# FluxML/Flux3D.jl

Measured on AMD Instinct MI355X. Metric: chamfer_point_pairs_per_sec, higher is better.
Workload: dtype f32

## Files before the change

### flux3d.jl_amd/csrc/chamfer.hip

```cpp
#include <cmath>

#include "nn1_common.h"

using namespace fx3d;

#ifdef FX3D_PROBE
__device__ unsigned long long g_probe[4096 * 16];
#define FX3D_PROBE_MARK(k)                                                                   \
    do {                                                                                     \
        if (threadIdx.x == 0 && blockIdx.x < 4096) {                                         \
            g_probe[blockIdx.x * 16 + (k)] = __builtin_readcyclecounter();                   \
            if ((k) == 0) g_probe[blockIdx.x * 16 + 13] = wall_clock64();                    \
            if ((k) == 12) g_probe[blockIdx.x * 16 + 14] = wall_clock64();                   \
        }                                                                                    \
    } while (0)
__device__ unsigned long long g_probe2[256 * 16];
#define FX3D_PROBE_MARK2(k) do { if (threadIdx.x == 0 && blockIdx.x < 256) g_probe2[blockIdx.x * 16 + (k)] = __builtin_readcyclecounter(); } while (0)
__device__ unsigned long long g_probe3[16 * 16 * 8];
#define FX3D_PROBE_MARKW(k) do { if ((threadIdx.x & 63) == 0 && blockIdx.x < 16) g_probe3[(blockIdx.x * 16 + (threadIdx.x >> 6)) * 8 + (k)] = __builtin_readcyclecounter(); } while (0)
#else
#define FX3D_PROBE_MARK(k) do { } while (0)
#define FX3D_PROBE_MARK2(k) do { } while (0)
#define FX3D_PROBE_MARKW(k) do { } while (0)
#endif

namespace {

__device__ __forceinline__ void load4pts(const float *__restrict__ base, int p0, float (&px)[4],
                                         float (&py)[4], float (&pz)[4]) {
    const float4 *s4 = reinterpret_cast<const float4 *>(base + (size_t)p0 * 3);
    const float4 f0 = s4[0], f1 = s4[1], f2 = s4[2];
    px[0] = f0.x; py[0] = f0.y; pz[0] = f0.z;
    px[1] = f0.w; py[1] = f1.x; pz[1] = f1.y;
    px[2] = f1.z; py[2] = f1.w; pz[2] = f2.x;
    px[3] = f2.y; py[3] = f2.z; pz[3] = f2.w;
}

typedef _Float16 h8 __attribute__((ext_vector_type(8)));
typedef float f32x16 __attribute__((ext_vector_type(16)));
#ifndef FX3D_HFIFO
#define FX3D_HFIFO 5
#endif
constexpr int kHFifo = FX3D_HFIFO;
#ifndef FX3D_HRUNS_FROM
#define FX3D_HRUNS_FROM 16
#endif
constexpr int kHRunsFrom = FX3D_HRUNS_FROM;
constexpr int kScanU = 2;
#ifndef FX3D_HRUNCAP
#define FX3D_HRUNCAP 384
#endif
constexpr int kHRunCap = FX3D_HRUNCAP;
constexpr int kHItemCap = 64 * kHFifo > kHRunCap ? 64 * kHFifo : kHRunCap;
constexpr int kHFarCap = 64;
#ifndef FX3D_HBLKTRACK
#define FX3D_HBLKTRACK 1
#endif
constexpr bool kHBlkTrack = FX3D_HBLKTRACK != 0;
constexpr int kHIdBits = kHBlkTrack ? 7 : 6;
static_assert(kHChunkMax / (32 * kHLT) <= 64, "lane-tile ids live in the six (block ids: seven) low mantissa bits of the tracked keys");
constexpr float kKeyUp = kHBlkTrack ? 0x1.2p-16f : 0x1.2p-17f;
constexpr float kPadF16 = 65504.0f;
__device__ const unsigned short kHilbertCell[512] = {
    0, 1, 65, 64, 72, 73, 9, 8, 16, 24, 88, 80, 81, 89, 25, 17, 18, 26, 27, 19, 83, 91, 90, 82, 74, 10, 11, 75, 67, 3, 2, 66,
    130, 194, 195, 131, 139, 203, 202, 138, 146, 154, 155, 147, 211, 219, 218, 210, 209, 217, 153, 145, 144, 152, 216, 208, 200, 201, 137, 136, 128, 129, 193, 192,
    256, 257, 265, 264, 328, 329, 321, 320, 384, 448, 456, 392, 393, 457, 449, 385, 386, 450, 451, 387, 395, 459, 458, 394, 330, 322, 323, 331, 267, 259, 258, 266,
    274, 282, 283, 275, 339, 347, 346, 338, 402, 466, 467, 403, 411, 475, 474, 410, 409, 473, 465, 401, 400, 464, 472, 408, 344, 345, 337, 336, 272, 273, 281, 280,
    288, 296, 297, 289, 353, 361, 360, 352, 416, 480, 481, 417, 425, 489, 488, 424, 432, 496, 504, 440, 441, 505, 497, 433, 369, 368, 376, 377, 313, 312, 304, 305,
    306, 307, 315, 314, 378, 379, 371, 370, 434, 498, 506, 442, 443, 507, 499, 435, 427, 491, 490, 426, 418, 482, 483, 419, 355, 363, 362, 354, 290, 298, 299, 291,
    227, 235, 171, 163, 162, 170, 234, 226, 225, 224, 160, 161, 169, 168, 232, 233, 241, 240, 248, 249, 185, 184, 176, 177, 178, 242, 250, 186, 187, 251, 243, 179,
    115, 51, 59, 123, 122, 58, 50, 114, 113, 112, 120, 121, 57, 56, 48, 49, 41, 40, 104, 105, 97, 96, 32, 33, 34, 42, 106, 98, 99, 107, 43, 35,
    36, 44, 108, 100, 101, 109, 45, 37, 38, 39, 103, 102, 110, 111, 47, 46, 54, 55, 63, 62, 126, 127, 119, 118, 117, 53, 61, 125, 124, 60, 52, 116,
    180, 244, 252, 188, 189, 253, 245, 181, 182, 183, 191, 190, 254, 255, 247, 246, 238, 239, 175, 174, 166, 167, 231, 230, 229, 237, 173, 165, 164, 172, 236, 228,
    292, 300, 301, 293, 357, 365, 364, 356, 420, 484, 485, 421, 429, 493, 492, 428, 436, 500, 508, 444, 445, 509, 501, 437, 373, 372, 380, 381, 317, 316, 308, 309,
    310, 311, 319, 318, 382, 383, 375, 374, 438, 502, 510, 446, 447, 511, 503, 439, 431, 495, 494, 430, 422, 486, 487, 423, 359, 367, 366, 358, 294, 302, 303, 295,
    287, 286, 278, 279, 343, 342, 350, 351, 415, 479, 471, 407, 406, 470, 478, 414, 413, 477, 476, 412, 404, 468, 469, 405, 341, 349, 348, 340, 276, 284, 285, 277,
    269, 261, 260, 268, 332, 324, 325, 333, 397, 461, 460, 396, 388, 452, 453, 389, 390, 454, 462, 398, 399, 463, 455, 391, 327, 326, 334, 335, 271, 270, 262, 263,
    199, 198, 134, 135, 143, 142, 206, 207, 215, 223, 159, 151, 150, 158, 222, 214, 213, 221, 220, 212, 148, 156, 157, 149, 141, 205, 204, 140, 132, 196, 197, 133,
    69, 5, 4, 68, 76, 12, 13, 77, 85, 93, 92, 84, 20, 28, 29, 21, 22, 30, 94, 86, 87, 95, 31, 23, 15, 14, 78, 79, 71, 70, 6, 7,
};
constexpr size_t kHScratchBytes = (kHThreads / 64) * (32 * 8 + kHItemCap * 2 + 32 * 3 * 4) + 64 * 32;

__device__ __forceinline__ float vmin(float a, float b) {
    float r;
    asm("v_min_f32 %0, %1, %2" : "=v"(r) : "v"(a), "v"(b));
    return r;
}

__device__ __forceinline__ void split2h(float v, _Float16 &h, _Float16 &l) {
    h = (_Float16)v;
    l = (_Float16)(v - (float)h);
}

constexpr float kBetaC = 0x1.1p-18f;
constexpr float kBandB1 = 1.0f + 18.0f * kBetaC + 0x1p-20f;
constexpr float kBandA = 22.3f * kBetaC + 0x1p-19f;
__device__ __forceinline__ void make_pieces(float cx, float cy, float cz, h8 &p0, h8 &p1) {
    _Float16 hx, lx, hy, ly, hz, lz, n1, n2, n3;
    split2h(cx, hx, lx); split2h(cy, hy, ly); split2h(cz, hz, lz);
    const float n0 = ((cx * cx) + (cy * cy)) + (cz * cz);
    const float n = n0 + kBetaC * n0;
    n1 = (_Float16)n;
    const float r1 = n - (float)n1;
    n2 = (_Float16)r1;
    n3 = (_Float16)(r1 - (float)n2);
    const _Float16 z = (_Float16)0.0f;
    p0 = h8{hx, hx, lx, hy, hy, ly, hz, hz};
    p1 = h8{lz, n1, n2, n3, lx, ly, lz, z};
}

template <bool WANT_IDX, bool SPLITFUSE = false, bool PRUNE = false>
__global__ __launch_bounds__(kHThreads, 4) void nn1_f16_kernel(Nn1Params p) {
    extern __shared__ __attribute__((aligned(16))) float lds[];
    __shared__ __attribute__((aligned(16))) float red[4 * 4 * (kHThreads / 64) + 16];
    __shared__ int nfar[2];
    __shared__ unsigned short farlist[kHFarCap];
    constexpr int QB = (kHThreads / 64) * 32;

    const int L = blockIdx.x;
    const int per_cloud = p.tiles * p.nsplit;
    const bool by_xcd = 2 * p.B >= 8;
// ... 12 lines not shown
    const int NCm = NC - ctail;
    const float *__restrict__ qb = (dir ? p.y : p.x) + (size_t)b * NQ * 3;
    const float *__restrict__ cb = (dir ? p.x : p.y) + (size_t)b * NC * 3;
    int32_t *idx_out = dir ? p.idx_y : p.idx_x;
    float *dmin_out = dir ? p.dmin_y : p.dmin_x;

    const int tid = threadIdx.x, lane = tid & 63;
    const int wv = __builtin_amdgcn_readfirstlane(tid >> 6);
    const int jq = lane & 31, hh = lane >> 5;
    const int CH = p.chunk;
    const int tpb = dir ? p.tpb_y : p.tpb;
    h8 *imgp = reinterpret_cast<h8 *>(lds);
    float4 *imgf = reinterpret_cast<float4 *>(lds);
    unsigned long long *wres = reinterpret_cast<unsigned long long *>(lds + 8 * (CH + 64));
    unsigned short *witems = reinterpret_cast<unsigned short *>(wres + (kHThreads / 64) * 32);
    float *wq = reinterpret_cast<float *>(witems + (kHThreads / 64) * kHItemCap);
    unsigned long long *qres = wres + wv * 32;
    unsigned short *items = witems + wv * kHItemCap;
    float *qtab = wq + wv * 96;
    const bool vec = (reinterpret_cast<uintptr_t>(cb) & 15) == 0;
    const bool one_shot = NCm <= CH;
    if (tid == 0) { nfar[0] = 0; nfar[1] = 0; }
    float qpre[3];
    {
        const int q0i = (tile * tpb) * QB + wv * 32 + jq;
        const int qc0 = q0i < NQ ? q0i : NQ - 1;
#pragma unroll
        for (int d = 0; d < 3; ++d) qpre[d] = qb[(size_t)qc0 * 3 + d];
    }
    if constexpr (PRUNE) {
        unsigned int *zc = reinterpret_cast<unsigned int *>(wres);
        for (int i = tid; i < 1040 + 16 * 256; i += kHThreads) zc[i] = 0u;
        int *gb = reinterpret_cast<int *>(wq + (kHThreads / 64) * 96) + 64 * 8;
        for (int i = tid; i < kHGroupsMax * 8; i += kHThreads) gb[i] = (i & 4) ? (int)0x80000000 : 0x7fffffff;
    }
    FX3D_PROBE_MARK(0);

    const bool own_chunk_only = p.nsplit > 1 && (long long)split * CH + (long long)p.nsplit * CH >= NCm;
    const int s_lo = own_chunk_only ? split * CH : 0;
    const int SN = own_chunk_only ? (NCm - s_lo < CH ? NCm - s_lo : CH) : NC;
    const float *__restrict__ sb = cb + (size_t)s_lo * 3;
    const bool parked = one_shot || own_chunk_only;
    float mu[3], cinf = 0.0f, varmax = 0.0f;
    float bxlo[3] = {0.f, 0.f, 0.f}, bxhi[3] = {0.f, 0.f, 0.f};
    bool allfin = true;
    {
        float mn[3] = {INFINITY, INFINITY, INFINITY}, mx[3] = {-INFINITY, -INFINITY, -INFINITY}, sm3[3] = {0.f, 0.f, 0.f};
        float sqt = 0.0f;
        const float pil[3] = {sb[0], sb[1], sb[2]};
        const int nsweep = (SN + kHThreads - 1) / kHThreads;
        for (int i0 = 0; i0 < nsweep; i0 += 4) {
            P3 v[4];
#pragma unroll
            for (int e = 0; e < 4; ++e) {
                const int pt = (i0 + e) * kHThreads + tid;
                v[e] = *reinterpret_cast<const P3 *>(sb + (size_t)(pt < SN ? pt : SN - 1) * 3);
            }
#pragma unroll
            for (int e = 0; e < 4; ++e) {
                const int pt = (i0 + e) * kHThreads + tid;
                mn[0] = fminf(mn[0], v[e].x); mx[0] = fmaxf(mx[0], v[e].x);
                mn[1] = fminf(mn[1], v[e].y); mx[1] = fmaxf(mx[1], v[e].y);
                mn[2] = fminf(mn[2], v[e].z); mx[2] = fmaxf(mx[2], v[e].z);
                if (pt < SN) {
                    sm3[0] = sm3[0] + v[e].x; sm3[1] = sm3[1] + v[e].y; sm3[2] = sm3[2] + v[e].z;
                    if (parked) imgf[((pt >> 5) * 2) * 32 + (pt & 31)] = float4{v[e].x, v[e].y, v[e].z, 0.0f};
                }
// ... 32 lines not shown
#undef NN1_ROW_MAX
#undef NN1_ROW_SUM
            const float lo3[3] = {lo4.x, lo4.y, lo4.z}, hi3[3] = {hi4.x, hi4.y, hi4.z}, st3[3] = {st4.x, st4.y, st4.z};
            float m3[3], ci = 0.0f, vm = st4.w / fmaxf(0.25f * (float)SN, 1.0f);
            bool fin = true;
#pragma unroll
            for (int d = 0; d < 3; ++d) {
                const float lo = lo3[d], hi = hi3[d], st = st3[d];
                m3[d] = fminf(fmaxf(st / (float)SN, lo), hi);
                const float off = st / (float)SN - pil[d];
                vm = vm - off * off;
                ci = fmaxf(ci, fmaxf(hi - m3[d], m3[d] - lo));
                fin = fin && fabsf(st) < INFINITY;
            }
            if (lane == 0) {
                float4 *o4 = reinterpret_cast<float4 *>(red) + 4 * (kHThreads / 64);
                o4[0] = float4{m3[0], m3[1], m3[2], ci * 1.000001f};
                o4[1] = float4{vm, fin ? 1.0f : 0.0f, 0.0f, 0.0f};
                if (PRUNE) { o4[2] = float4{lo3[0], lo3[1], lo3[2], 0.0f}; o4[3] = float4{hi3[0], hi3[1], hi3[2], 0.0f}; }
            }
        }
        __syncthreads();
        {
            const float4 *o4 = reinterpret_cast<const float4 *>(red) + 4 * (kHThreads / 64);
            const float4 a = o4[0], b2 = o4[1];
            mu[0] = a.x; mu[1] = a.y; mu[2] = a.z; cinf = a.w;
            varmax = b2.x; allfin = b2.y != 0.0f;
            if (PRUNE) {
                const float4 l4 = o4[2], h4 = o4[3];
                bxlo[0] = l4.x; bxlo[1] = l4.y; bxlo[2] = l4.z; bxhi[0] = h4.x; bxhi[1] = h4.y; bxhi[2] = h4.z;
            }
        }
    }
    float rng = cinf;
    if (allfin && cinf < 1.0e16f && 3.0f * cinf * cinf > kRobustGate * varmax) {
        const float4 r = robust_range3<kHThreads, false>(sb, SN, parked, imgf, red, mu[0], mu[1], mu[2], cinf);
        mu[0] = r.x; mu[1] = r.y; mu[2] = r.z; rng = r.w;
    }
    const bool sane = allfin && cinf < 1.0e16f;
    float sc = 1.0f;
    if (sane && rng > 1.0e-30f) {
        int e;
        (void)frexpf(rng, &e);
        sc = ldexpf(1.0f, 7 - e);
    }
    auto uni = [](float v) { return __builtin_bit_cast(float, __builtin_amdgcn_readfirstlane(__builtin_bit_cast(int, v))); };
    mu[0] = uni(mu[0]); mu[1] = uni(mu[1]); mu[2] = uni(mu[2]); sc = uni(sc); rng = uni(rng); cinf = uni(cinf);
    const bool has_far = sane && rng < cinf;
    int fslot = 0;
    auto pieces = [&](float x, float y, float z, int pt, h8 &p0, h8 &p1) {
        const float sx = (x - mu[0]) * sc, sy = (y - mu[1]) * sc, sz = (z - mu[2]) * sc;
        if (!has_far) { make_pieces(sx, sy, sz, p0, p1); return; }
        const bool far = !(fmaxf(fmaxf(fabsf(sx), fabsf(sy)), fabsf(sz)) < 128.0f);
        make_pieces(far ? 0.f : sx, far ? 0.f : sy, far ? 0.f : sz, p0, p1);
        if (far) {
            p1[7] = (_Float16)kPadF16;
            const int f = atomicAdd(&nfar[fslot], 1);
            if (f < kHFarCap) farlist[f] = (unsigned short)pt;
        }
    };

    [[maybe_unused]] float4 *cs = nullptr, *qsw = nullptr;
    [[maybe_unused]] bool sorted_c = false;
    [[maybe_unused]] int qwlen = 0;
    [[maybe_unused]] float4 *boxes = nullptr;
    if constexpr (PRUNE) {
        cs = p.pscr + (size_t)blockIdx.x * p.pscr_stride;
        qsw = cs + kHChunkMax;
        boxes = reinterpret_cast<float4 *>(wq + (kHThreads / 64) * 96);
        unsigned int *ccnt = reinterpret_cast<unsigned int *>(wres);
        unsigned int *qtot = ccnt + 520;
        unsigned int *qwh = qtot + 520;
        const bool last_t = tile == (dir ? p.tiles_y : p.tiles_x) - 1;
        const int qw0 = tile * tpb * QB;
        const int qw1 = last_t || qw0 + tpb * QB > NQ ? NQ : qw0 + tpb * QB;
        qwlen = qw1 - qw0;
        const int cnt = NCm;
        const bool do_sort = sane && cnt >= 512;
        const bool sorted_q = do_sort && NQ <= 4 * kHThreads;
        P3 qv[4];
        if (sorted_q) {
#pragma unroll
            for (int e = 0; e < 4; ++e) {
                const int qp = 256 * wv + 64 * e + lane;
                qv[e] = *reinterpret_cast<const P3 *>(qb + (size_t)(qp < NQ ? qp : NQ - 1) * 3);
            }
        }
        FX3D_PROBE_MARK2(0);
        int *gbox = reinterpret_cast<int *>(boxes + 64 * 2);
        auto group_box = [&](int wrow, float x, float y, float z) {
            int *g = gbox + (wrow >> 5) * 8;
            atomicMin(g + 0, fkey((x - mu[0]) * sc)); atomicMin(g + 1, fkey((y - mu[1]) * sc)); atomicMin(g + 2, fkey((z - mu[2]) * sc));
            atomicMax(g + 4, fkey((x - mu[0]) * sc)); atomicMax(g + 5, fkey((y - mu[1]) * sc)); atomicMax(g + 6, fkey((z - mu[2]) * sc));
        };
        if (do_sort) {
            float4 cv[4];
#pragma unroll
            for (int e = 0; e < 4; ++e) {
                const int pt = e * kHThreads + tid;
                cv[e] = float4{0.f, 0.f, 0.f, 0.f};
                if (pt < cnt) cv[e] = imgf[((pt >> 5) * 2) * 32 + (pt & 31)];
            }
            FX3D_PROBE_MARK2(1);
            float inv[3], off[3], cfl[3], cfh[3];
#pragma unroll
            for (int d = 0; d < 3; ++d) {
                const float fr = has_far ? 0.125f * rng : 128.0f / sc;
                const float flo = fmaxf(bxlo[d], mu[d] - fr), fhi = fminf(bxhi[d], mu[d] + fr);
                inv[d] = fhi > flo ? 8.0f / (fhi - flo) : 0.0f;
                off[d] = -flo * inv[d];
                cfl[d] = flo; cfh[d] = fhi;
            }
            auto cell = [&](float x, float y, float z) -> unsigned int {
                const unsigned int ux = (unsigned int)(int)fminf(fmaxf(__builtin_fmaf(x, inv[0], off[0]), 0.0f), 7.0f);
                const unsigned int uy = (unsigned int)(int)fminf(fmaxf(__builtin_fmaf(y, inv[1], off[1]), 0.0f), 7.0f);
                const unsigned int uz = (unsigned int)(int)fminf(fmaxf(__builtin_fmaf(z, inv[2], off[2]), 0.0f), 7.0f);
                return ux | (uy << 3) | (uz << 6);
            };

            unsigned int ccr[4], qcr[4];
            auto count_cells = [&](bool valid, unsigned int t, auto &&add) -> unsigned int {
                unsigned int rank = 0u;
                bool mine = valid;
                const unsigned int tn = (unsigned int)__builtin_amdgcn_update_dpp((int)~t, (int)t, 0x111, 0xF, 0xF, false);
                if (__builtin_popcountll(__ballot(valid && t == tn)) >= 8) {
                    unsigned long long rem = __ballot(valid);
                    for (int it = 0; it < 12 && rem; ++it) {
                        const unsigned int t0 = (unsigned int)__builtin_amdgcn_readlane((int)t, __builtin_ctzll(rem));
                        const unsigned long long grp = __ballot(mine && t == t0);
                        rem &= ~grp;
                        if (__builtin_popcountll(grp) < 4) continue;
                        unsigned int base = 0u;
                        if ((int)lane == __builtin_ctzll(grp)) base = add(t0, (unsigned int)__builtin_popcountll(grp));
                        base = (unsigned int)__builtin_amdgcn_readlane((int)base, __builtin_ctzll(grp));
                        if (mine && t == t0) {
                            rank = base + __builtin_amdgcn_mbcnt_hi((unsigned int)(grp >> 32), __builtin_amdgcn_mbcnt_lo((unsigned int)grp, 0u));
                            mine = false;
                        }
                    }
                }
                if (mine) rank = add(t, 1u);
                return rank;
            };
#pragma unroll
            for (int e = 0; e < 4; ++e) {
                const int pt = e * kHThreads + tid;
                const unsigned int t = pt < cnt ? cell(cv[e].x, cv[e].y, cv[e].z) : 0u;
                ccr[e] = (t << 16) | count_cells(pt < cnt, t, [&](unsigned int c, unsigned int n) { return atomicAdd(&ccnt[c], n); });
            }
            int *qbb = reinterpret_cast<int *>(boxes + 64 * 2 + kHGroupsMax * 2 - 2);
            if (sorted_q) {
                int kl[3] = {0x7fffffff, 0x7fffffff, 0x7fffffff}, kh[3] = {(int)0x80000000, (int)0x80000000, (int)0x80000000};
#pragma unroll
                for (int e = 0; e < 4; ++e) {
                    const int qp = 256 * wv + 64 * e + lane;
                    if (qp < NQ) {
                        const int k3[3] = {fkey(qv[e].x), fkey(qv[e].y), fkey(qv[e].z)};
#pragma unroll
                        for (int d = 0; d < 3; ++d) { kl[d] = kl[d] < k3[d] ? kl[d] : k3[d]; kh[d] = kh[d] > k3[d] ? kh[d] : k3[d]; }
                    }
                }
#pragma unroll
                for (int d = 0; d < 3; ++d) {
                    int a = row_mm_key<false>(kl[d]), b2 = row_mm_key<true>(kh[d]);
                    a = imm<false>(a, dpp_keepi<0x142, 0xA>(a)); a = imm<false>(a, dpp_keepi<0x143, 0xC>(a));
                    b2 = imm<true>(b2, dpp_keepi<0x142, 0xA>(b2)); b2 = imm<true>(b2, dpp_keepi<0x143, 0xC>(b2));
                    if (lane == 63) { atomicMin(qbb + d, a); atomicMax(qbb + 4 + d, b2); }
                }
            }
            FX3D_PROBE_MARK2(2);
            __syncthreads();
            FX3D_PROBE_MARK2(3);
            float qinv[3] = {0.f, 0.f, 0.f}, qoff[3] = {0.f, 0.f, 0.f};
            if (sorted_q) {
                const float ext = fmaxf(fmaxf(cfh[0] - cfl[0], cfh[1] - cfl[1]), cfh[2] - cfl[2]);
#pragma unroll
                for (int d = 0; d < 3; ++d) {
                    const float ql = fkey_inv(qbb[d]), qh = fkey_inv(qbb[4 + d]);
                    const float grow = qh - ql > 4.0f * ext ? 0.25f * ext : ext;
                    const float lo = fmaxf(ql, cfl[d] - grow), hi = fminf(qh, cfh[d] + grow);
                    qinv[d] = hi > lo && hi - lo < INFINITY ? 8.0f / (hi - lo) : 0.0f;
                    qoff[d] = qinv[d] != 0.0f ? -lo * qinv[d] : 0.0f;
                }
            }
            auto qcell = [&](float x, float y, float z) -> unsigned int {
                const unsigned int ux = (unsigned int)(int)fminf(fmaxf(__builtin_fmaf(x, qinv[0], qoff[0]), 0.0f), 7.0f);
                const unsigned int uy = (unsigned int)(int)fminf(fmaxf(__builtin_fmaf(y, qinv[1], qoff[1]), 0.0f), 7.0f);
                const unsigned int uz = (unsigned int)(int)fminf(fmaxf(__builtin_fmaf(z, qinv[2], qoff[2]), 0.0f), 7.0f);
                return ux | (uy << 3) | (uz << 6);
            };
            auto curve_scan = [&](unsigned int *a) {
                unsigned int tc[8];
                {
                    const uint4 h = *reinterpret_cast<const uint4 *>(kHilbertCell + 8 * lane);
                    tc[0] = h.x & 0xffffu; tc[1] = h.x >> 16; tc[2] = h.y & 0xffffu; tc[3] = h.y >> 16;
                    tc[4] = h.z & 0xffffu; tc[5] = h.z >> 16; tc[6] = h.w & 0xffffu; tc[7] = h.w >> 16;
                }
                unsigned int c8[8], tot = 0u;
#pragma unroll
                for (int k = 0; k < 8; ++k) { c8[k] = a[tc[k]]; tot += c8[k]; }
                unsigned int inc = tot;
#pragma unroll
                for (int o = 1; o < 64; o <<= 1) {
                    const unsigned int v = __shfl_up(inc, o, 64);
                    if (lane >= o) inc += v;
                }
                unsigned int run = inc - tot;
#pragma unroll
                for (int k = 0; k < 8; ++k) { a[tc[k]] = run; run += c8[k]; }
            };
            if (wv == 0) curve_scan(ccnt);
            if (sorted_q) {
#pragma unroll
                for (int e = 0; e < 4; ++e) {
                    const int qp = 256 * wv + 64 * e + lane;
                    const unsigned int t = qp < NQ ? qcell(qv[e].x, qv[e].y, qv[e].z) : 0u;
                    qcr[e] = (t << 16) | count_cells(qp < NQ, t, [&](unsigned int c, unsigned int n) {
                                 const unsigned int sh = 16u * (c & 1u);
                                 const unsigned int old = atomicAdd(&qwh[wv * 256 + (c >> 1)], n << sh);
                                 atomicAdd(&qtot[c], n);
                                 return (old >> sh) & 0xffffu;
                             });
                }
            }
            FX3D_PROBE_MARK2(4);
            __syncthreads();
            FX3D_PROBE_MARK2(5);
#pragma unroll
            for (int e = 0; e < 4; ++e) {
                const int pt = e * kHThreads + tid;
                if (pt < cnt) {
                    const int pos = (int)(ccnt[ccr[e] >> 16] + (ccr[e] & 0xffffu));
                    imgf[((pos >> 5) * 2) * 32 + (pos & 31)] = float4{cv[e].x, cv[e].y, cv[e].z, __builtin_bit_cast(float, pt)};
                }
            }
            sorted_c = true;
            if (sorted_q) {
                if (wv == 1) {
                    curve_scan(qtot);
                } else if (wv >= 2 && wv < 6) {
                    const int w2 = tid - 128;
                    unsigned int run = 0u;
#pragma unroll
                    for (int w = 0; w < 16; ++w) {
                        const unsigned int v = qwh[w * 256 + w2];
                        qwh[w * 256 + w2] = run;
                        run += v;
                    }
                }
            }
            FX3D_PROBE_MARK2(6);
            __syncthreads();
            FX3D_PROBE_MARK2(7);
            if (sorted_q) {
#pragma unroll
                for (int e = 0; e < 4; ++e) {
                    const int qp = 256 * wv + 64 * e + lane;
                    if (qp < NQ) {
                        const unsigned int t = qcr[e] >> 16;
                        const int rank = (int)(qtot[t] + ((qwh[wv * 256 + (t >> 1)] >> (16u * (t & 1u))) & 0xffffu) + (qcr[e] & 0xffffu));
                        if (rank >= qw0 && rank < qw1) {
                            qsw[rank - qw0] = float4{qv[e].x, qv[e].y, qv[e].z, __builtin_bit_cast(float, qp)};
                            group_box(rank - qw0, qv[e].x, qv[e].y, qv[e].z);
                        }
                    }
                }
            }
        }
        if (!sorted_q) {
            for (int q0 = qw0 + wv * 64; q0 < qw1; q0 += kHThreads) {
                const int qp = q0 + lane;
                const P3 r = *reinterpret_cast<const P3 *>(qb + (size_t)(qp < qw1 ? qp : qw1 - 1) * 3);
                if (qp < qw1) qsw[qp - qw0] = float4{r.x, r.y, r.z, __builtin_bit_cast(float, qp)};
                const int kx = fkey((r.x - mu[0]) * sc), ky = fkey((r.y - mu[1]) * sc), kz = fkey((r.z - mu[2]) * sc);
                const int lx = row_mm_key<false>(kx), ly = row_mm_key<false>(ky), lz = row_mm_key<false>(kz);
                const int hx = row_mm_key<true>(kx), hy = row_mm_key<true>(ky), hz = row_mm_key<true>(kz);
                if ((lane & 15) == 0 && qp < qw1) {
                    int *g = gbox + ((qp - qw0) >> 5) * 8;
                    atomicMin(g + 0, lx); atomicMin(g + 1, ly); atomicMin(g + 2, lz);
                    atomicMax(g + 4, hx); atomicMax(g + 5, hy); atomicMax(g + 6, hz);
                }
            }
        }
        FX3D_PROBE_MARK2(8);
    }
    FX3D_PROBE_MARK(1);

    const float cm2 = 3.0f * (fminf(cinf * sc, 128.0f) * fminf(cinf * sc, 128.0f));
    float qr[3], da = 0.0f;
    float da_far = 0.0f;
    [[maybe_unused]] float dpr = INFINITY;
    bool qfin = true;
    int qi = 0;
    bool qok = true;
    h8 bq;
    double acc = 0.0;

    const int jfirst = split * CH, jstep = p.nsplit * CH;
    for (int j0 = jfirst; j0 < NCm; j0 += jstep) {
        const int cnt = (NCm - j0) < CH ? (NCm - j0) : CH;
        const int cnt_pad = (cnt + 32 * kHLT - 1) / (32 * kHLT) * (32 * kHLT);
        if (j0 > jfirst) __syncthreads();
        if constexpr (PRUNE) {
            for (int tl = tid >> 4; tl * 64 < cnt_pad + 64; tl += kHThreads / 16) {
                float4 r4[4];
#pragma unroll
                for (int k = 0; k < 4; ++k) {
                    const int pt = tl * 64 + k * 16 + (tid & 15);
                    r4[k] = float4{0.f, 0.f, 0.f, 0.f};
                    if (pt < cnt) r4[k] = imgf[((pt >> 5) * 2) * 32 + (pt & 31)];
                }
                float lo3[3] = {INFINITY, INFINITY, INFINITY}, hi3[3] = {-INFINITY, -INFINITY, -INFINITY};
#pragma unroll
                for (int k = 0; k < 4; ++k) {
                    const int pt = tl * 64 + k * 16 + (tid & 15), i0 = ((pt >> 5) * 2) * 32 + (pt & 31);
                    h8 p0, p1;
                    if (pt < cnt) {
                        pieces(r4[k].x, r4[k].y, r4[k].z, pt, p0, p1);
                        const int id = sorted_c ? __builtin_bit_cast(int, r4[k].w) : j0 + pt;
                        cs[pt] = float4{r4[k].x, r4[k].y, r4[k].z, __builtin_bit_cast(float, id)};
                        const float b3[3] = {(r4[k].x - mu[0]) * sc, (r4[k].y - mu[1]) * sc, (r4[k].z - mu[2]) * sc};
#pragma unroll
                        for (int d = 0; d < 3; ++d) { lo3[d] = vmin(lo3[d], b3[d]); hi3[d] = -vmin(-hi3[d], -b3[d]); }
                    } else {
                        make_pieces(0.f, 0.f, 0.f, p0, p1);
                        p1[7] = (_Float16)kPadF16;
                    }
                    imgp[i0] = p0;
                    imgp[i0 + 32] = p1;
                }
                float bl[3], bh[3];
#pragma unroll
                for (int d = 0; d < 3; ++d) { bl[d] = fkey_inv(row_mm_key<false>(fkey(lo3[d]))); bh[d] = fkey_inv(row_mm_key<true>(fkey(hi3[d]))); }
                if ((tid & 15) == 0 && tl < 64) {
                    boxes[tl * 2] = float4{bl[0], bl[1], bl[2], 0.0f};
                    boxes[tl * 2 + 1] = float4{bh[0], bh[1], bh[2], 0.0f};
                }
            }
        } else
        for (int pt = tid; pt < cnt_pad + 64; pt += kHThreads) {
            const int i0 = ((pt >> 5) * 2) * 32 + (pt & 31);
            h8 p0, p1;
            if (pt < cnt) {
                if (parked) {
                    const float4 r = imgf[i0];
                    pieces(r.x, r.y, r.z, pt, p0, p1);
                } else {
                    const P3 r = *reinterpret_cast<const P3 *>(cb + (size_t)(j0 + pt) * 3);
                    pieces(r.x, r.y, r.z, pt, p0, p1);
                }
            } else {
                make_pieces(0.f, 0.f, 0.f, p0, p1);
                p1[7] = (_Float16)kPadF16;
            }
            imgp[i0] = p0;
            imgp[i0 + 32] = p1;
        }
        __syncthreads();
        FX3D_PROBE_MARK(j0 == jfirst ? 2 : 6);
        FX3D_PROBE_MARKW(0);

        const int nf = nfar[fslot];
        if (tid == 0) nfar[fslot ^ 1] = 0;
        fslot ^= 1;
        const bool far_ok = nf <= kHFarCap;
        const bool last_tile = tile == (dir ? p.tiles_y : p.tiles_x) - 1;
        for (int tp = 0; tp < tpb || (last_tile && one_shot); ++tp) {
            if ((tile * tpb + tp) * QB >= NQ) break;
            if constexpr (PRUNE) {
                if (tp * QB + wv * 32 >= qwlen) continue;
            }
            if (j0 == jfirst) {
                qi = (tile * tpb + tp) * QB + wv * 32 + jq;
                if constexpr (PRUNE) {
                    const int wpos = tp * QB + wv * 32 + jq;
                    const float4 q4 = qsw[wpos < qwlen ? wpos : qwlen - 1];
                    qr[0] = q4.x; qr[1] = q4.y; qr[2] = q4.z;
                    qi = wpos < qwlen ? __builtin_bit_cast(int, q4.w) : NQ;
                } else if (tp == 0) {
#pragma unroll
                    for (int d = 0; d < 3; ++d) qr[d] = qpre[d];
                } else {
                    const int qc1 = qi < NQ ? qi : NQ - 1;
#pragma unroll
                    for (int d = 0; d < 3; ++d) qr[d] = qb[(size_t)qc1 * 3 + d];
                }
                float m0 = -2.0f * ((qr[0] - mu[0]) * sc), m1 = -2.0f * ((qr[1] - mu[1]) * sc), m2 = -2.0f * ((qr[2] - mu[2]) * sc);
                float S = (fabsf(m0) + fabsf(m1)) + fabsf(m2);
                float sq = 1.0f, fl_s = 0.0f;
                if (S >= 3.0e4f && S < 0x1p28f) {
                    int e;
                    (void)frexpf(S, &e);
                    sq = ldexpf(1.0f, 14 - e);
                    m0 *= sq; m1 *= sq; m2 *= sq; S *= sq;
                    fl_s = 0x1p-15f;
                }
                qok = S < 3.0e4f;
                qfin = fabsf(qr[0]) + fabsf(qr[1]) + fabsf(qr[2]) < INFINITY;
                const float qn = 0.25f * ((m0 * m0 + m1 * m1) + m2 * m2) / sq;
                da = kBandA * qn + 0x1p-24f * (S + 4.0f) + fl_s;
                {
                    const float c2 = sq * cm2;
                    da_far = 2.1f * kBetaC * c2 + 2.0f * kBetaC * sqrtf(qn * c2) + 0x1p-19f * qn + 0x1p-24f * (S + 4.0f) + fl_s;
                }
                if constexpr (PRUNE) {
                    dpr = qok && sq == 1.0f ? qn + 2.0f * kBetaC * (cm2 + qn) + 0x1p-23f * (S + 4.0f) : INFINITY;
                }
                _Float16 hx, lx, hy, ly, hz, lz;
                split2h(qok ? m0 : 0.f, hx, lx); split2h(qok ? m1 : 0.f, hy, ly); split2h(qok ? m2 : 0.f, hz, lz);
                const _Float16 one = (_Float16)sq, pad = (_Float16)kPadF16;
                bq = hh == 0 ? h8{hx, lx, hx, hy, ly, hy, hz, lz} : h8{hz, one, one, one, lx, ly, lz, pad};
                if (hh == 0) {
                    qres[jq] = ~0ull;
                    qtab[jq * 3 + 0] = qr[0]; qtab[jq * 3 + 1] = qr[1]; qtab[jq * 3 + 2] = qr[2];
                }
            }

            float tm = INFINITY, fk[kHFifo];
#pragma unroll
            for (int s = 0; s < kHFifo; ++s) fk[s] = INFINITY;
            const unsigned int keymask = ~((1u << kHIdBits) - 1u);

            static_assert(kHLT == 2, "the rotation below is written for lane tiles of two blocks");
            const int nblk = cnt_pad / 32;
            f32x16 zero;
#pragma unroll
            for (int r = 0; r < 16; ++r) zero[r] = 0.0f;
#define NN1_FOLD(ACC, FIRST)                                                                                         \
            {                                                                                                        \
                const float t0 = min3f(ACC[0], ACC[1], ACC[2]), t1 = min3f(ACC[3], ACC[4], ACC[5]);                  \
                const float t2 = min3f(ACC[6], ACC[7], ACC[8]), t3 = min3f(ACC[9], ACC[10], ACC[11]);                \
                const float t4 = min3f(ACC[12], ACC[13], ACC[14]);                                                   \
// ... 15 lines not shown
            __builtin_amdgcn_s_setprio(0);                                                                           \
            ISSUE = __builtin_amdgcn_mfma_f32_32x32x16_f16(an, bq, zero, 0, 0, 0);                                   \
            an = pa[(OFF) * 64];                                                                                     \
            __builtin_amdgcn_s_setprio(1);                                                                           \
            NN1_CLOSE(FOLD, ODD, lt)                                                                                 \
            if (ODD) ++lt;
            if constexpr (!PRUNE) {
            const h8 *pa = imgp + hh * 32 + jq;
            f32x16 acc0, acc1, acc2;
            h8 an = pa[0];
            acc0 = __builtin_amdgcn_mfma_f32_32x32x16_f16(an, bq, zero, 0, 0, 0); an = pa[1 * 64];
            acc1 = __builtin_amdgcn_mfma_f32_32x32x16_f16(an, bq, zero, 0, 0, 0); an = pa[2 * 64];
            pa += 3 * 64;
            int lt = 0;
            int nb = 2;
            for (; nb + 6 <= nblk; nb += 6) {
                NN1_STEP(acc2, acc0, 0, 0) NN1_STEP(acc0, acc1, 1, 1) NN1_STEP(acc1, acc2, 0, 2)
                NN1_STEP(acc2, acc0, 1, 3) NN1_STEP(acc0, acc1, 0, 4) NN1_STEP(acc1, acc2, 1, 5)
                pa += 6 * 64;
            }
            if (nblk - nb == 4) {
                NN1_STEP(acc2, acc0, 0, 0) NN1_STEP(acc0, acc1, 1, 1) NN1_STEP(acc1, acc2, 0, 2) NN1_STEP(acc2, acc0, 1, 3)
                NN1_CLOSE(acc1, 0, lt) NN1_CLOSE(acc2, 1, lt)
            } else if (nblk - nb == 2) {
                NN1_STEP(acc2, acc0, 0, 0) NN1_STEP(acc0, acc1, 1, 1)
                NN1_CLOSE(acc2, 0, lt) NN1_CLOSE(acc0, 1, lt)
            } else {
                NN1_CLOSE(acc0, 0, lt) NN1_CLOSE(acc1, 1, lt)
            }
            } else {
            const int nltp = nblk / kHLT;
            float bd = INFINITY;
            {
                const int4 *gq = reinterpret_cast<const int4 *>(boxes + 64 * 2) + (tp * (kHThreads / 64) + wv) * 2;
                const int4 gl = gq[0], gh = gq[1];
                const float qlx = fkey_inv(gl.x), qly = fkey_inv(gl.y), qlz = fkey_inv(gl.z);
                const float qhx = fkey_inv(gh.x), qhy = fkey_inv(gh.y), qhz = fkey_inv(gh.z);
                if (lane < nltp) {
                    const float4 lo = boxes[lane * 2], hi = boxes[lane * 2 + 1];
                    const float gx = fmaxf(fmaxf(lo.x - qhx, qlx - hi.x), 0.0f), gy = fmaxf(fmaxf(lo.y - qhy, qly - hi.y), 0.0f);
                    const float gz = fmaxf(fmaxf(lo.z - qhz, qlz - hi.z), 0.0f);
                    bd = (gx * gx + gy * gy) + gz * gz;
                }
            }
            const unsigned long long all_lt = nltp >= 64 ? ~0ull : (1ull << nltp) - 1ull;
            unsigned long long todo = all_lt, done = 0ull;
            if (sorted_c) {
                todo = __ballot(bd == 0.0f);
                if (!todo) {
                    const float bmin = wave_min_f(bd);
                    todo = bmin < INFINITY ? __ballot(bd == bmin) : all_lt;
                }
            }
            const h8 *pbase = imgp + hh * 32 + jq;
            for (int phase = 0; phase < 2; ++phase) {
                if (phase == 1) {
                    if (done == all_lt) break;
                    const float kb = fk[0];
                    const float bb = __builtin_fmaf(fabsf(kb), kKeyUp, kb);
                    const float dj = fminf(bb, __shfl_xor(bb, 32, 64)) + dpr;
                    const float ucut = wave_max_f(__builtin_fmaf(dj, 1.0f + 0x1p-9f, 0x1p-8f));
                    const bool keep = !(bd > ucut) || !(dj == dj);
                    todo = (__ballot(!(dj == dj)) ? all_lt : __ballot(keep)) & all_lt & ~done;
                    if (!todo) break;
                }
                done |= todo;
                unsigned long long mk = todo;
                int nrem = __builtin_popcountll(mk) - 1;
// ... 322 lines not shown
                        const float *src = cb + (size_t)jc * 3;
                        const float cc3[3] = {src[0], src[1], src[2]};
                        atomicMin(&qres[qs], ((unsigned long long)dist_key(sqd<3>(qq, cc3)) << 32) | (unsigned int)jc);
                    }
                }
            }
            FX3D_PROBE_MARK(tp == 0 ? 4 : 8);
            FX3D_PROBE_MARKW(tp == 0 ? 2 : 4);

            if (j0 + jstep >= NCm) {
                __builtin_amdgcn_s_waitcnt(0xc07f);
                __builtin_amdgcn_wave_barrier();
                if (hh == 0) {
                    const unsigned long long r = qres[jq];
                    const float dd = __builtin_bit_cast(float, (unsigned int)(r >> 32));
                    const int ii = (int)(unsigned int)r;
                    if (p.nsplit > 1) {
                        unsigned long long *gp = &p.gres[((size_t)split * 2 * p.B + c) * p.qstride + qi];
                        if (qi < NQ) {
                            if (SPLITFUSE) __hip_atomic_store(gp, r, __ATOMIC_RELAXED, __HIP_MEMORY_SCOPE_AGENT);
                            else *gp = r;
                        }
                    } else if (qi < NQ) {
                        if (WANT_IDX && idx_out) idx_out[(size_t)b * NQ + qi] = ii;
                        if (dmin_out) dmin_out[(size_t)b * NQ + qi] = dd;
                        acc += (double)dd;
                    }
                }
                __builtin_amdgcn_wave_barrier();
            }
        }
    }
    FX3D_PROBE_MARK(11);
    if (SPLITFUSE && p.nsplit > 1) {
        __shared__ int s_last;
        FX3D_PROBE_MARK2(10);
        asm volatile("s_waitcnt vmcnt(0)" ::: "memory");
        FX3D_PROBE_MARK2(11);
        __syncthreads();
        FX3D_PROBE_MARK2(12);
        const int ns = (NC + CH - 1) / CH < p.nsplit ? (NC + CH - 1) / CH : p.nsplit;
        if (tid == 0) {
            const unsigned int t = (unsigned int)c * (unsigned int)p.tiles + (unsigned int)tile;
            unsigned int *ctr = p.ticket + (t / 15u) * 16u + 1u + t % 15u;
            const unsigned int old = __hip_atomic_fetch_add(ctr, 1u, __ATOMIC_RELAXED, __HIP_MEMORY_SCOPE_AGENT);
            s_last = old == (unsigned int)ns - 1u;
            if (s_last) __hip_atomic_store(ctr, 0u, __ATOMIC_RELAXED, __HIP_MEMORY_SCOPE_AGENT);
            FX3D_PROBE_MARK2(13);
        }
        __syncthreads();
        if (!s_last) return;
        FX3D_PROBE_MARK(6);
        acc = 0.0;
        const int qend = (tile + 1) * tpb * QB < NQ ? (tile + 1) * tpb * QB : NQ;
        constexpr int kQ = 1, kS = 16;
        for (int q0 = tile * tpb * QB + tid; q0 < qend; q0 += kQ * kHThreads) {
          unsigned long long rr[kQ][kS];
#pragma unroll
          for (int u = 0; u < kQ; ++u)
#pragma unroll
            for (int sp = 0; sp < kS; ++sp) {
                const int q = q0 + u * kHThreads < qend ? q0 + u * kHThreads : q0;
                const int spc = sp < ns ? sp : ns - 1;
                rr[u][sp] = __hip_atomic_load(&p.gres[((size_t)spc * 2 * p.B + c) * p.qstride + q], __ATOMIC_RELAXED, __HIP_MEMORY_SCOPE_AGENT);
            }
#ifdef FX3D_PROBE
// ... 57 lines not shown
#pragma unroll
            for (int e = 0; e < 4; ++e) o[e] = p.gres[((size_t)(sp + e < ns ? sp + e : 0) * 2 * p.B + c) * p.qstride + qi];
#pragma unroll
            for (int e = 0; e < 4; ++e) r = o[e] < r ? o[e] : r;
        }
        const float dd = __builtin_bit_cast(float, (unsigned int)(r >> 32));
        int32_t *idx_out = dir ? p.idx_y : p.idx_x;
        float *dmin_out = dir ? p.dmin_y : p.dmin_x;
        if (idx_out) idx_out[(size_t)b * NQ + qi] = (int)(unsigned int)r;
        if (dmin_out) dmin_out[(size_t)b * NQ + qi] = dd;
        acc = (double)dd;
    }
    if (p.partials) {
        __shared__ double sm[kThreads / 64];
        const double tot = block_sum<kThreads>(acc, sm);
        if (!p.ticket) {
            if (threadIdx.x == 0) p.partials[(size_t)c * tiles_f + blockIdx.x] = tot;
            return;
        }
        if (threadIdx.x < 64) {
            const FinalizeArgs fa{reinterpret_cast<unsigned long long *>(p.partials), p.ticket, p.nvalid, p.B, tiles_f, p.tiles_x, p.tiles_y,
                                  p.sums_out, p.loss_out, p.N, p.M, p.Bg, p.w1, p.w2};
            (void)fused_finalize_wave0(fa, (size_t)c * tiles_f + blockIdx.x, tot, (int)threadIdx.x);
        }
    }
}

}

namespace fx3d {

size_t nn1_f16_lds_bytes(int chunk) { return (size_t)chunk * 8 * sizeof(float) + kHScratchBytes; }

constexpr size_t kHBoxBytes = 64 * 2 * sizeof(float4) + kHGroupsMax * 32;

template <bool WANT_IDX>
static fx3d_status launch_f16(const Nn1Params &p, int grid, size_t lds_bytes, hipStream_t st) {
    void (*const kfn)(Nn1Params) = p.pscr ? &nn1_f16_kernel<WANT_IDX, false, true>
                                   : p.fuse_split ? &nn1_f16_kernel<WANT_IDX, true> : &nn1_f16_kernel<WANT_IDX, false>;
    const size_t box = p.pscr ? kHBoxBytes : 0;
    const fx3d_status arc = ensure_dynamic_lds(reinterpret_cast<const void *>(kfn), (int)(nn1_f16_lds_bytes(kHChunkMax) + box), "nn1_f16_kernel");
    if (arc != FX3D_OK) return arc;
    hipLaunchKernelGGL(kfn, dim3(grid), dim3(kHThreads), lds_bytes + box, st, p);
    FX3D_LAUNCH_CHECK();
    return FX3D_OK;
}

fx3d_status nn1_f16_launch(const Nn1Params &p, int grid, size_t lds_bytes, hipStream_t st) {
    return p.idx_x || p.idx_y ? launch_f16<true>(p, grid, lds_bytes, st) : launch_f16<false>(p, grid, lds_bytes, st);
}

fx3d_status nn1_split_finalize_launch(const Nn1Params &p, int tiles_f, hipStream_t st) {
    hipLaunchKernelGGL(nn1_split_finalize_kernel, dim3(tiles_f, 2 * p.B), dim3(kThreads), 0, st, p, tiles_f);
    FX3D_LAUNCH_CHECK();
    return FX3D_OK;
}

}
```

### flux3d.jl_amd/csrc/chamfer_host.hip

```cpp
#include <cmath>
#include <cstdlib>

#include "nn1_common.h"

using namespace fx3d;

namespace {

struct FinalizeParams {
    const double *partials;
    int B, tiles, tiles_x, tiles_y;
    double *sums;
    float *loss;
    int N, M, D;
    long long Bg;
    float w1, w2;
};

__global__ __launch_bounds__(kThreads) void chamfer_finalize_partials_kernel(FinalizeParams f) {
    __shared__ double sm[kThreads / 64];
    double tot[2];
    for (int dir = 0; dir < 2; ++dir) {
        const int nt = dir ? f.tiles_y : f.tiles_x;
        const long long n = (long long)f.B * nt;
// ... 142 lines not shown
                t = t > thr ? t : thr;
                const long long tmax = tiles_a > tiles_b ? tiles_a : tiles_b;
                t += 1.0 * (double)((2ll * B * tmax + ncu - 1) / ncu - 1);
                if (t < bt - 1e-9) { bt = t; pl.tpb = ta; pl.tpb_y = tb; }
            }
    }
    const bool fold = b_split == 1 && maxc <= b_chunk;
    auto ntiles = [&](int nq, int tpb) {
        const int per = 512 * tpb;
        int t = ceil_div(nq, per);
        if (fold && t > 1 && nq - (t - 1) * per <= kHTail) --t;
        return t;
    };
    pl.tiles_x = ntiles(N, pl.tpb);
    pl.tiles_y = ntiles(M, pl.tpb_y);
    pl.tiles = pl.tiles_x > pl.tiles_y ? pl.tiles_x : pl.tiles_y;
    pl.grid = clouds8 * 8 * pl.tiles * pl.nsplit;
    if (2 * B < 8) pl.grid = 2 * B * pl.tiles * pl.nsplit;
    return pl;
}

Nn1Kernel plan_kernel(const Plan &pl, int D) {
    if (D != 2 && D != 3) return NN1_GENERIC;
    return pl.variant == 3 ? NN1_F16 : pl.variant == 4 ? NN1_TINY : NN1_SMALL_D;
}
const char *plan_kernel_name(const Plan &pl, int D) {
    static const char *const names[] = {"generic", "small_d", "tiny", "f16"};
    return names[plan_kernel(pl, D)];
}

int prune_rows_per_block(const Plan &pl, int N, int M, int D) {
    const int maxc = N > M ? N : M;
    if (plan_kernel(pl, D) != NN1_F16 || pl.nsplit != 1 || pl.tail != 0 || maxc > pl.chunk || maxc < 1024 || !opt(OPT_NN1_PRUNE)) return 0;
    if ((pl.tpb > pl.tpb_y ? pl.tpb : pl.tpb_y) * 16 + 2 > kHGroupsMax - 1) return 0;
    if ((pl.tpb < pl.tpb_y ? pl.tpb : pl.tpb_y) < 2) return 0;
    return kHChunkMax + (pl.tpb > pl.tpb_y ? pl.tpb : pl.tpb_y) * 512 + kHTail;
}

struct Workspace {
    int tiles;
    size_t sums, gres, need, pscr, total;
};
Workspace workspace_layout(const Plan &pl, int N, int M, int B, int D) {
    Workspace w{};
    const int maxq = N > M ? N : M;
    w.tiles = pl.nsplit > 1 ? ceil_div(maxq, kThreads) : pl.tiles;
    w.sums = (size_t)2 * B * w.tiles * sizeof(double);
    w.gres = w.sums + 2 * sizeof(double);
    w.need = w.gres + (pl.nsplit > 1 ? (size_t)pl.nsplit * 2 * B * maxq * sizeof(unsigned long long) : 0);
    w.pscr = (w.need + 255) & ~(size_t)255;
    const size_t ps = (size_t)prune_rows_per_block(pl, N, M, D) * pl.grid * sizeof(float4);
    w.total = ps ? w.pscr + ps : w.need;
    return w;
}

constexpr long long kSplitFuseMax = 255;

fx3d_status run_nn1(Nn1Params p, int D, const Plan &pl, hipStream_t st) {
    p.tiles = pl.tiles; p.tiles_x = pl.tiles_x; p.tiles_y = pl.tiles_y; p.chunk = pl.chunk;
    p.tpb = pl.tpb; p.tpb_y = pl.tpb_y;
    p.tail = pl.tail;
    p.nsplit = p.gres ? pl.nsplit : 1;
    p.fuse_split = p.gres && p.ticket ? 1 : 0;
    p.pscr_stride = p.pscr ? prune_rows_per_block(pl, p.N, p.M, D) : 0;
    if (!p.pscr_stride) p.pscr = nullptr;
    const Nn1Kernel k = plan_kernel(pl, D);
    ProfileScope prof("nn1", st);
// ... 144 lines not shown
```

### flux3d.jl_amd/csrc/nn1_common.h

```cpp
#pragma once
#include "fx3d_common.h"

namespace fx3d {

constexpr int kThreads = 256;
constexpr int kTile = 32;
constexpr int kChunkMax = 4096;

struct Nn1Params {
    const float *x;
    const float *y;
    int N, M, B;
    int32_t *idx_x, *idx_y;
    float *dmin_x, *dmin_y;
    double *partials;
    int tiles;
    int tiles_x, tiles_y;
    int chunk;
    int tpb;
    int tpb_y;
    unsigned int *ticket;
    unsigned int nvalid;
    double *sums_out;
    float *loss_out;
// ... 26 lines not shown
    for (int d = 1; d < DIM; ++d) {
        float t = q[d] - c[d];
        s = s + t * t;
    }
    return s;
}

__device__ __forceinline__ bool fless(float a, float b) { return (a < b) || (b != b && a == a); }
__device__ __forceinline__ unsigned int dist_key(float d) { return d != d ? 0x7fc00000u : __builtin_bit_cast(unsigned int, d); }

template <int DIM>
__device__ __forceinline__ void nn1_scan_isless(const float (&q)[DIM], const float *__restrict__ cb, int NC, float &best, int &bi) {
    float c0[DIM];
#pragma unroll
    for (int d = 0; d < DIM; ++d) c0[d] = cb[d];
    best = sqd<DIM>(q, c0);
    bi = 0;
    for (int j = 1; j < NC; ++j) {
        float cc[DIM];
#pragma unroll
        for (int d = 0; d < DIM; ++d) cc[d] = cb[(size_t)j * DIM + d];
        const float dd = sqd<DIM>(q, cc);
        if (fless(dd, best)) { best = dd; bi = j; }
    }
}

constexpr int kHThreads = 1024;
#ifndef FX3D_HLT
#define FX3D_HLT 2
#endif
constexpr int kHLT = FX3D_HLT;
constexpr int kHChunkMax = 4096;
constexpr int kHTail = 64;
constexpr int kHGroupsMax = 8 * 16 + 2 + 1;

constexpr int kTyThreads = 256;
constexpr int kTyQ = 16;
constexpr int kTySl = 16;
constexpr int kTyG = 16;

__device__ __forceinline__ float chamfer_loss_from_sums(double sa, double sb, int N, int M, int D,
                                                        long long Bg, float w1, float w2) {
    const float dA = (float)(sa / ((double)D * (double)N * (double)Bg)) * 3.0f;
    const float dB = (float)(sb / ((double)D * (double)M * (double)Bg)) * 3.0f;
    return (w1 * dA) + (w2 * dB);
}

#if defined(__HIP_DEVICE_COMPILE__) && !defined(__gfx950__)
#error "nn1_common.h: the relaxed-atomic + s_waitcnt hand-off between blocks is validated on gfx950 only (see the note above)"
#endif
struct FinalizeArgs {
    unsigned long long *pp;
    unsigned int *ticket;
    unsigned int nvalid;
    int B, stride, tiles_x, tiles_y;
    double *sums_out;
    float *loss_out;
    int N, M;
    long long Bg;
    float w1, w2;
};
__device__ __forceinline__ int fused_finalize_wave0(const FinalizeArgs &f, size_t slot, double tot, int lane) {
    int last = 0;
    if (lane == 0) {
        __hip_atomic_store(&f.pp[slot], __builtin_bit_cast(unsigned long long, tot), __ATOMIC_RELAXED, __HIP_MEMORY_SCOPE_AGENT);
        asm volatile("s_waitcnt vmcnt(0)" ::: "memory");
        const unsigned int old = __hip_atomic_fetch_add(f.ticket, 1u, __ATOMIC_RELAXED, __HIP_MEMORY_SCOPE_AGENT);
// ... 34 lines not shown
```

Measured before the change: 14580 billion.

## Compute per-half-wave query boxes with lane reductions instead of LDS atomics

```diff
diff --git a/flux3d.jl_amd/csrc/chamfer.hip b/flux3d.jl_amd/csrc/chamfer.hip
--- a/flux3d.jl_amd/csrc/chamfer.hip
+++ b/flux3d.jl_amd/csrc/chamfer.hip
@@ -22,6 +22,11 @@
 #define FX3D_PROBE_MARK(k) do { } while (0)
 #define FX3D_PROBE_MARK2(k) do { } while (0)
 #define FX3D_PROBE_MARKW(k) do { } while (0)
+#endif
+#ifdef FX3D_PROBE_STOP
+#define FX3D_PROBE_STOP_AT(k) do { if (FX3D_PROBE_STOP == (k)) return; } while (0)
+#else
+#define FX3D_PROBE_STOP_AT(k) do { } while (0)
 #endif
 
 namespace {
@@ -87,6 +92,18 @@
     return r;
 }
 
+template <bool MAX>
+__device__ __forceinline__ int half_mm_key(int k) {
+    k = row_mm_key<MAX>(k);
+    return imm<MAX>(__builtin_amdgcn_readlane(k, 0), __builtin_amdgcn_readlane(k, 16));
+}
+
+__device__ __forceinline__ float vmax(float a, float b) {
+    float r;
+    asm("v_max_f32 %0, %1, %2" : "=v"(r) : "v"(a), "v"(b));
+    return r;
+}
+
 __device__ __forceinline__ void split2h(float v, _Float16 &h, _Float16 &l) {
     h = (_Float16)v;
     l = (_Float16)(v - (float)h);
@@ -165,7 +182,7 @@
         unsigned int *zc = reinterpret_cast<unsigned int *>(wres);
         for (int i = tid; i < 1040 + 16 * 256; i += kHThreads) zc[i] = 0u;
         int *gb = reinterpret_cast<int *>(wq + (kHThreads / 64) * 96) + 64 * 8;
-        for (int i = tid; i < kHGroupsMax * 8; i += kHThreads) gb[i] = (i & 4) ? (int)0x80000000 : 0x7fffffff;
+        if (tid < 8) gb[tid] = (tid & 4) ? (int)0x80000000 : 0x7fffffff;
     }
     FX3D_PROBE_MARK(0);
 
@@ -264,6 +281,7 @@
             }
         }
     }
+    FX3D_PROBE_STOP_AT(1);
     float rng = cinf;
     if (allfin && cinf < 1.0e16f && 3.0f * cinf * cinf > kRobustGate * varmax) {
         const float4 r = robust_range3<kHThreads, false>(sb, SN, parked, imgf, red, mu[0], mu[1], mu[2], cinf);
@@ -319,12 +337,6 @@
             }
         }
         FX3D_PROBE_MARK2(0);
-        int *gbox = reinterpret_cast<int *>(boxes + 64 * 2);
-        auto group_box = [&](int wrow, float x, float y, float z) {
-            int *g = gbox + (wrow >> 5) * 8;
-            atomicMin(g + 0, fkey((x - mu[0]) * sc)); atomicMin(g + 1, fkey((y - mu[1]) * sc)); atomicMin(g + 2, fkey((z - mu[2]) * sc));
-            atomicMax(g + 4, fkey((x - mu[0]) * sc)); atomicMax(g + 5, fkey((y - mu[1]) * sc)); atomicMax(g + 6, fkey((z - mu[2]) * sc));
-        };
         if (do_sort) {
             float4 cv[4];
 #pragma unroll
@@ -380,7 +392,7 @@
                 const unsigned int t = pt < cnt ? cell(cv[e].x, cv[e].y, cv[e].z) : 0u;
                 ccr[e] = (t << 16) | count_cells(pt < cnt, t, [&](unsigned int c, unsigned int n) { return atomicAdd(&ccnt[c], n); });
             }
-            int *qbb = reinterpret_cast<int *>(boxes + 64 * 2 + kHGroupsMax * 2 - 2);
+            int *qbb = reinterpret_cast<int *>(boxes + 64 * 2);
             if (sorted_q) {
                 int kl[3] = {0x7fffffff, 0x7fffffff, 0x7fffffff}, kh[3] = {(int)0x80000000, (int)0x80000000, (int)0x80000000};
 #pragma unroll
@@ -403,6 +415,7 @@
             FX3D_PROBE_MARK2(2);
             __syncthreads();
             FX3D_PROBE_MARK2(3);
+            FX3D_PROBE_STOP_AT(2);
             float qinv[3] = {0.f, 0.f, 0.f}, qoff[3] = {0.f, 0.f, 0.f};
             if (sorted_q) {
                 const float ext = fmaxf(fmaxf(cfh[0] - cfl[0], cfh[1] - cfl[1]), cfh[2] - cfl[2]);
@@ -458,6 +471,7 @@
             FX3D_PROBE_MARK2(4);
             __syncthreads();
             FX3D_PROBE_MARK2(5);
+            FX3D_PROBE_STOP_AT(3);
 #pragma unroll
             for (int e = 0; e < 4; ++e) {
                 const int pt = e * kHThreads + tid;
@@ -484,6 +498,7 @@
             FX3D_PROBE_MARK2(6);
             __syncthreads();
             FX3D_PROBE_MARK2(7);
+            FX3D_PROBE_STOP_AT(4);
             if (sorted_q) {
 #pragma unroll
                 for (int e = 0; e < 4; ++e) {
@@ -491,10 +506,7 @@
                     if (qp < NQ) {
                         const unsigned int t = qcr[e] >> 16;
                         const int rank = (int)(qtot[t] + ((qwh[wv * 256 + (t >> 1)] >> (16u * (t & 1u))) & 0xffffu) + (qcr[e] & 0xffffu));
-                        if (rank >= qw0 && rank < qw1) {
-                            qsw[rank - qw0] = float4{qv[e].x, qv[e].y, qv[e].z, __builtin_bit_cast(float, qp)};
-                            group_box(rank - qw0, qv[e].x, qv[e].y, qv[e].z);
-                        }
+                        if (rank >= qw0 && rank < qw1) qsw[rank - qw0] = float4{qv[e].x, qv[e].y, qv[e].z, __builtin_bit_cast(float, qp)};
                     }
                 }
             }
@@ -504,19 +516,12 @@
                 const int qp = q0 + lane;
                 const P3 r = *reinterpret_cast<const P3 *>(qb + (size_t)(qp < qw1 ? qp : qw1 - 1) * 3);
                 if (qp < qw1) qsw[qp - qw0] = float4{r.x, r.y, r.z, __builtin_bit_cast(float, qp)};
-                const int kx = fkey((r.x - mu[0]) * sc), ky = fkey((r.y - mu[1]) * sc), kz = fkey((r.z - mu[2]) * sc);
-                const int lx = row_mm_key<false>(kx), ly = row_mm_key<false>(ky), lz = row_mm_key<false>(kz);
-                const int hx = row_mm_key<true>(kx), hy = row_mm_key<true>(ky), hz = row_mm_key<true>(kz);
-                if ((lane & 15) == 0 && qp < qw1) {
-                    int *g = gbox + ((qp - qw0) >> 5) * 8;
-                    atomicMin(g + 0, lx); atomicMin(g + 1, ly); atomicMin(g + 2, lz);
-                    atomicMax(g + 4, hx); atomicMax(g + 5, hy); atomicMax(g + 6, hz);
-                }
             }
         }
         FX3D_PROBE_MARK2(8);
     }
     FX3D_PROBE_MARK(1);
+    FX3D_PROBE_STOP_AT(5);
 
     const float cm2 = 3.0f * (fminf(cinf * sc, 128.0f) * fminf(cinf * sc, 128.0f));
     float qr[3], da = 0.0f;
@@ -534,7 +539,13 @@
         const int cnt_pad = (cnt + 32 * kHLT - 1) / (32 * kHLT) * (32 * kHLT);
         if (j0 > jfirst) __syncthreads();
         if constexpr (PRUNE) {
-            for (int tl = tid >> 4; tl * 64 < cnt_pad + 64; tl += kHThreads / 16) {
+            if (tid >= kHThreads - 64) {
+                const int pt = cnt_pad + lane, i0 = ((pt >> 5) * 2) * 32 + (pt & 31);
+                const _Float16 z = (_Float16)0.0f;
+                imgp[i0] = h8{z, z, z, z, z, z, z, z};
+                imgp[i0 + 32] = h8{z, z, z, z, z, z, z, (_Float16)kPadF16};
+            }
+            for (int tl = tid >> 4; tl * 64 < cnt_pad; tl += kHThreads / 16) {
                 float4 r4[4];
 #pragma unroll
                 for (int k = 0; k < 4; ++k) {
@@ -553,7 +564,7 @@
                         cs[pt] = float4{r4[k].x, r4[k].y, r4[k].z, __builtin_bit_cast(float, id)};
                         const float b3[3] = {(r4[k].x - mu[0]) * sc, (r4[k].y - mu[1]) * sc, (r4[k].z - mu[2]) * sc};
 #pragma unroll
-                        for (int d = 0; d < 3; ++d) { lo3[d] = vmin(lo3[d], b3[d]); hi3[d] = -vmin(-hi3[d], -b3[d]); }
+                        for (int d = 0; d < 3; ++d) { lo3[d] = vmin(lo3[d], b3[d]); hi3[d] = vmax(hi3[d], b3[d]); }
                     } else {
                         make_pieces(0.f, 0.f, 0.f, p0, p1);
                         p1[7] = (_Float16)kPadF16;
@@ -590,6 +601,7 @@
         }
         __syncthreads();
         FX3D_PROBE_MARK(j0 == jfirst ? 2 : 6);
+        FX3D_PROBE_STOP_AT(6);
         FX3D_PROBE_MARKW(0);
 
         const int nf = nfar[fslot];
@@ -620,16 +632,18 @@
                 float m0 = -2.0f * ((qr[0] - mu[0]) * sc), m1 = -2.0f * ((qr[1] - mu[1]) * sc), m2 = -2.0f * ((qr[2] - mu[2]) * sc);
                 float S = (fabsf(m0) + fabsf(m1)) + fabsf(m2);
                 float sq = 1.0f, fl_s = 0.0f;
+                float rsq = 1.0f;
                 if (S >= 3.0e4f && S < 0x1p28f) {
                     int e;
                     (void)frexpf(S, &e);
                     sq = ldexpf(1.0f, 14 - e);
+                    rsq = ldexpf(1.0f, e - 14);
                     m0 *= sq; m1 *= sq; m2 *= sq; S *= sq;
                     fl_s = 0x1p-15f;
                 }
                 qok = S < 3.0e4f;
                 qfin = fabsf(qr[0]) + fabsf(qr[1]) + fabsf(qr[2]) < INFINITY;
-                const float qn = 0.25f * ((m0 * m0 + m1 * m1) + m2 * m2) / sq;
+                const float qn = 0.25f * ((m0 * m0 + m1 * m1) + m2 * m2) * rsq;
                 da = kBandA * qn + 0x1p-24f * (S + 4.0f) + fl_s;
                 {
                     const float c2 = sq * cm2;
@@ -711,8 +725,12 @@
             const int nltp = nblk / kHLT;
             float bd = INFINITY;
             {
-                const int4 *gq = reinterpret_cast<const int4 *>(boxes + 64 * 2) + (tp * (kHThreads / 64) + wv) * 2;
-                const int4 gl = gq[0], gh = gq[1];
+                int4 gl, gh;
+                {
+                    const int kx = fkey((qr[0] - mu[0]) * sc), ky = fkey((qr[1] - mu[1]) * sc), kz = fkey((qr[2] - mu[2]) * sc);
+                    gl.x = half_mm_key<false>(kx); gl.y = half_mm_key<false>(ky); gl.z = half_mm_key<false>(kz);
+                    gh.x = half_mm_key<true>(kx); gh.y = half_mm_key<true>(ky); gh.z = half_mm_key<true>(kz);
+                }
                 const float qlx = fkey_inv(gl.x), qly = fkey_inv(gl.y), qlz = fkey_inv(gl.z);
                 const float qhx = fkey_inv(gh.x), qhy = fkey_inv(gh.y), qhz = fkey_inv(gh.z);
                 if (lane < nltp) {
@@ -1101,6 +1119,7 @@
         }
     }
     FX3D_PROBE_MARK(11);
+    FX3D_PROBE_STOP_AT(7);
     if (SPLITFUSE && p.nsplit > 1) {
         __shared__ int s_last;
         FX3D_PROBE_MARK2(10);
@@ -1224,7 +1243,7 @@
 
 size_t nn1_f16_lds_bytes(int chunk) { return (size_t)chunk * 8 * sizeof(float) + kHScratchBytes; }
 
-constexpr size_t kHBoxBytes = 64 * 2 * sizeof(float4) + kHGroupsMax * 32;
+constexpr size_t kHBoxBytes = 64 * 2 * sizeof(float4) + 32;
 
 template <bool WANT_IDX>
 static fx3d_status launch_f16(const Nn1Params &p, int grid, size_t lds_bytes, hipStream_t st) {
diff --git a/flux3d.jl_amd/csrc/chamfer_host.hip b/flux3d.jl_amd/csrc/chamfer_host.hip
--- a/flux3d.jl_amd/csrc/chamfer_host.hip
+++ b/flux3d.jl_amd/csrc/chamfer_host.hip
@@ -198,7 +198,6 @@
 int prune_rows_per_block(const Plan &pl, int N, int M, int D) {
     const int maxc = N > M ? N : M;
     if (plan_kernel(pl, D) != NN1_F16 || pl.nsplit != 1 || pl.tail != 0 || maxc > pl.chunk || maxc < 1024 || !opt(OPT_NN1_PRUNE)) return 0;
-    if ((pl.tpb > pl.tpb_y ? pl.tpb : pl.tpb_y) * 16 + 2 > kHGroupsMax - 1) return 0;
     if ((pl.tpb < pl.tpb_y ? pl.tpb : pl.tpb_y) < 2) return 0;
     return kHChunkMax + (pl.tpb > pl.tpb_y ? pl.tpb : pl.tpb_y) * 512 + kHTail;
 }
diff --git a/flux3d.jl_amd/csrc/nn1_common.h b/flux3d.jl_amd/csrc/nn1_common.h
--- a/flux3d.jl_amd/csrc/nn1_common.h
+++ b/flux3d.jl_amd/csrc/nn1_common.h
@@ -82,7 +82,6 @@
 constexpr int kHLT = FX3D_HLT;
 constexpr int kHChunkMax = 4096;
 constexpr int kHTail = 64;
-constexpr int kHGroupsMax = 8 * 16 + 2 + 1;
 
 constexpr int kTyThreads = 256;
 constexpr int kTyQ = 16;
```

Result: no change. 14690 billion (median of 5 runs) (+0.8%).
